# a-rtemis99/hpc_suffix_array

Measured on AMD Instinct MI355X. Metric: suffixes sorted/sec + ms/doubling-round, 1 GiB input at 1/2/4/8 MI355X, higher is better.
Workload: dtype u32

## Files before the change

### hpc_suffix_array_amd/_native.py

```python
from __future__ import annotations

import ctypes
import os
import subprocess

PKG_DIR = os.path.dirname(os.path.abspath(__file__))
LIB_PATH = os.path.join(PKG_DIR, "lib", "libsa_hip.so")
LIB_PATH = os.environ.get("SA_LIB_PATH", LIB_PATH)
CSRC = os.path.join(PKG_DIR, "csrc")

SA_MAX_ROUNDS = 64
KERNEL_KINDS = ["init", "hist_first", "hist_keys", "scan", "scatter_first", "scatter_keys",
                "heads", "heads_scan", "rerank", "seg_count", "seg_scan", "seg_write", "alphabet", "pack",
                "sort_u", "windows", "local_sort", "pivot_keys", "pivot_count", "pivot_write"]
SCHEDULE_PACKED = 0
SCHEDULE_REFERENCE = 1
ROUND1_AUTO = 0
ROUND1_LSD = 1
ROUND1_BUCKETED = 2
SA_K_COUNT = len(KERNEL_KINDS)
FIND_AUTO = 0
FIND_LANE = 1
FIND_WAVE = 2
FIND_LANE_MAX = 3584
# ... 5 lines not shown
LOCATE_TILE = 2048
LOCATE_ORDERS = {"text": 0, "sa": LOCATE_SA_ORDER}
MEM_INFO = 3
MEM_TOO_MANY = 1
MEM_LANE = 1
MEM_WAVE = 2
MEM_MODES = {"auto": 0, "lane": MEM_LANE, "wave": MEM_WAVE}

DROPIN_SYMBOLS = ["create_suffix_array", "destroy_suffix_array", "build_suffix_array",
                  "build_lcp_array", "find_longest_repeated_substring", "is_valid_suffix_array"]
EXT_SYMBOLS = ["sa_context_create", "sa_context_destroy", "sa_context_set_debug", "sa_workspace_bytes", "sa_build_device",
               "sa_build_ex", "sa_check_device", "sa_check", "sa_lcp_device", "sa_lcp", "sa_generate_text_device",
               "sa_alphabet_device", "sa_pack_keys_device", "sa_sort_pairs_device", "sa_scatter_u64_device",
               "sa_gather_u64_device", "sa_running_max_i64_device", "sa_inclusive_sum_i64_device",
               "sa_count_below_u64_device", "sa_select_u8_device",
               "sa_find_device", "sa_find", "sa_find_ex",
               "sa_match_device", "sa_matching_stats_device", "sa_match", "sa_matching_stats",
               "sa_bwt_device", "sa_bwt", "sa_inverse_device", "sa_inverse",
               "sa_locate_device", "sa_locate",
               "sa_mems_device", "sa_mems",
               "sa_dist_begin", "sa_dist_cuts", "sa_dist_plan_cuts", "sa_dist_reserve", "sa_dist_release", "sa_dist_round1", "sa_dist_req_count", "sa_dist_req_fill",
               "sa_dist_answer", "sa_dist_refine",
               "sa_last_error", "sa_host_syncs", "sa_device_count", "sa_version", "sa_struct_size"]


class SAError(RuntimeError):
    """A libsa_hip entry point returned an error code."""


DEBUG_FLAGS = {"no_cmp": 0x1, "no_pk8": 0x2, "no_pad": 0x4, "pad_overflow": 0x8, "no_fast32": 0x10,
               "no_pivot": 0x20, "perm_always": 0x40, "no_xq": 0x80, "xq_overflow": 0x100,
               "no_tied": 0x200, "no_key1_round": 0x400, "no_eonly": 0x800,
               "eonly": 0x1000, "fast32_small": 0x2000, "no_round2_fused": 0x4000,
               "ls_one_wg": 0x8000, "no_alpha_sample": 0x10000, "alpha_sample_small": 0x20000}


def debug_bits(names) -> int:
    bits = 0
    for x in names or ():
        if x not in DEBUG_FLAGS:
            raise ValueError(f"unknown debug flag {x!r} (one of {sorted(DEBUG_FLAGS)})")
        bits |= DEBUG_FLAGS[x]
    return bits


class SaOpts(ctypes.Structure):
    _fields_ = [("profile", ctypes.c_int32), ("schedule", ctypes.c_int32), ("init_chars", ctypes.c_int32),
                ("radix", ctypes.c_int32), ("round1", ctypes.c_int32), ("debug", ctypes.c_uint32),
                ("span_extra", ctypes.c_int32), ("tune", ctypes.c_int32)]


class SaStats(ctypes.Structure):
    _fields_ = [
        ("rounds", ctypes.c_int32),
        ("n_kinds", ctypes.c_int32),
        ("total_ms", ctypes.c_double),
        ("h2d_ms", ctypes.c_double),
        ("d2h_ms", ctypes.c_double),
        ("round_ms", ctypes.c_double * SA_MAX_ROUNDS),
        ("distinct", ctypes.c_uint64 * SA_MAX_ROUNDS),
        ("passes", ctypes.c_int32 * SA_MAX_ROUNDS),
        ("sorted_n", ctypes.c_uint64 * SA_MAX_ROUNDS),
        ("prefix_len", ctypes.c_uint64 * SA_MAX_ROUNDS),
        ("schedule", ctypes.c_int32),
        ("init_chars", ctypes.c_int32),
        ("sigma", ctypes.c_int32),
        ("sparse_ranks", ctypes.c_int32),
# ... 219 lines not shown
```

### hpc_suffix_array_amd/csrc/sa_build.hip

```cpp
#include <hip/hip_runtime.h>

#include <algorithm>
#include <atomic>
#include <chrono>
#include <cstdarg>
#include <cstdio>
#include <cstdlib>
#include <cstring>
#include <mutex>
#include <string>
#include <thread>
#include <vector>

#include "../../include/sa_hip.h"

#ifndef SA_ALPHA_GRID
#define SA_ALPHA_GRID 2048
#endif

#include "sa_bucket.h"
#include "sa_check.h"
#include "sa_kernels.h"
#include "sa_lcp.h"
#include "sa_limits.h"
// ... 1238 lines not shown
    const int r1 = opts ? opts->round1 : SA_ROUND1_AUTO;
    bool bucketed = false;
    auto plan_round1 = [&](bool sampled, bool* complete) -> int {
        SA_HIP(hipMemsetAsync(c->alpha, 0, 8 * 4, s));
        tm.begin(SA_K_ALPHABET);
        if (sampled) {
            const bool first4k = (c->dbg & SA_DEBUG_ALPHA_SAMPLE_SMALL) != 0;
            const uint64_t nb = alpha_text_blocks(n), ns = alpha_sample_blocks(n, first4k);
            hipLaunchKernelGGL(k_alphabet_sample, dim3((uint32_t)std::min<uint64_t>(ns, 2ull * (uint32_t)c->cus)),
                               dim3(kBlock), 0, s, d_text, n, nb, ns, c->alpha);
            add_bytes(st, SA_K_ALPHABET, alpha_sample_bytes(n, first4k));
        } else {
            const uint32_t grid = (uint32_t)std::min<uint64_t>((n + kBlock * 16 - 1) / (kBlock * 16), SA_ALPHA_GRID);
            hipLaunchKernelGGL(k_alphabet, dim3(grid), dim3(kBlock), 0, s, d_text, n, c->alpha);
            add_bytes(st, SA_K_ALPHABET, n);
        }
        tm.end();
        SA_HIP(hipGetLastError());
        SA_HIP(hipMemcpyAsync(h_alpha, c->alpha, 8 * 4, hipMemcpyDeviceToHost, s));
        SA_HIP(hipMemcpyAsync(h_tail, d_text + (n - tail_n), tail_n, hipMemcpyDeviceToHost, s));
        SA_HIP(host_sync(s));
        *complete = true;
        for (uint32_t t = 0; t < tail_n; ++t) {
            const uint32_t x = h_tail[t];
            if (!((h_alpha[x >> 5] >> (x & 31)) & 1u)) *complete = false;
            h_alpha[x >> 5] |= 1u << (x & 31);
        }
        sigma = 0;
        for (int b = 0; b < 256; ++b) h_code[b] = ((h_alpha[b >> 5] >> (b & 31)) & 1u) ? (uint16_t)(++sigma) : 0;
        SA_HIP(hipMemcpyAsync(c->code, h_code, 256 * 2, hipMemcpyHostToDevice, s));
        c->dna = sigma == 4 && h_code['A'] && h_code['C'] && h_code['G'] && h_code['T'];
        K = choose_chars(sigma, n, opts ? opts->init_chars : 0);
        Kb = (opts && opts->init_chars > 0) || sigma <= 1 ? K : min_chars(sigma, n);
        bucketed = plan_bucketed(sigma, n, Kb, r1, c->radix, &bp, 1, (c->dbg & SA_DEBUG_NO_CMP) ? 0 : 1);
        if (bucketed && bp.bs.cmp && short_suffix_ties(h_tail, n, tail_n, h_code, sigma, bp.bs.s, bp.bs.R))
            bucketed = plan_bucketed(sigma, n, Kb, r1, c->radix, &bp, 1, 0);
        const bool force_eonly = (c->dbg & SA_DEBUG_EONLY) != 0;
        if (bucketed && bp.bs.cmp == 1 && ((sigma & (sigma - 1)) != 0 || force_eonly) &&
            !(c->dbg & SA_DEBUG_NO_EONLY)) {
            const uint32_t hb = bp.bs.bb - kLoBits;
            BucketPlan b2;
            if ((force_eonly || !plan_pk8(bp, hb, c->dbg, true)) && plan_bucketed(sigma, n, Kb, r1, c->radix, &b2, 1, 2) &&
                (force_eonly || plan_pk8(b2, hb, c->dbg, true)) &&
                !short_suffix_ties(h_tail, n, tail_n, h_code, sigma, b2.bs.s, b2.bs.R, b2.K))
                bp = b2;
        }
        return SA_OK;
    };
    bool sampled = !(c->dbg & SA_DEBUG_NO_ALPHA_SAMPLE) &&
                   (n >= kPadMinN || (c->dbg & SA_DEBUG_ALPHA_SAMPLE_SMALL)) && c->radix == 0 && r1 != SA_ROUND1_LSD;
    bool refuted = false;
    uint64_t* keys1 = nullptr;
    uint32_t ksh1 = 0;
    uint32_t P = 0;
    bool fused = false;
    bool r1_pivot = false;
    uint64_t D = 0, m = 0, G = 0;
    uint64_t seg1[3] = {0, 0, 0};
    int r2 = 0;
    for (;;) {
        bool complete = true;
        rc = plan_round1(sampled, &complete);
        if (rc) return rc;
        if (sampled && !(bucketed && complete)) {
            SA_TRACE("packed: sampled alphabet (sigma=%u) not kept: %s", sigma,
                     complete ? "round 1 is not bucketed" : "the tail holds another symbol");
            sampled = false;
            continue;
        }
        c->samples_pending = false;
        if (!bucketed) break;
        bool done = false;
        c->alpha_prove = sampled && sigma < 256;
        c->alpha_refuted = false;
        rc = round1_bucketed(c, d_text, n, d_sa, bp, full_range(bp, n), s, tm, st, &done, &fused, seg1, &ksh1, true,
// ... 1057 lines not shown
```

### hpc_suffix_array_amd/csrc/sa_round1.h

```cpp
#pragma once

#ifndef SA_HIST_WPC
#define SA_HIST_WPC 64
#endif
#ifndef SA_REC_STRIPED
#define SA_REC_STRIPED 1
#endif
#ifndef SA_BB_EXTRA
#define SA_BB_EXTRA 0
#endif
#ifndef SA_ITEMS_A
#define SA_ITEMS_A 12
#endif
#ifndef SA_TEXT_BLOCK
#define SA_TEXT_BLOCK 512
#endif
#ifndef SA_LIST_BLOCK
#define SA_LIST_BLOCK 1024
#endif


#ifndef SA_SEG_BLOCK
#define SA_SEG_BLOCK 1024
#endif
// ... 26 lines not shown
    const uint32_t e = ((uint32_t)c->tune >> 8) & 0xFFu;
    const uint32_t v = e ? e : 8u;
    return v >= 8 ? 8u : v >= 4 ? 4u : v >= 2 ? 2u : 1u;
}

__global__ __launch_bounds__(kLoRadix) void k_sum_rows(const uint32_t* __restrict__ in, uint32_t rows,
                                                       uint32_t* __restrict__ out) {
    uint32_t t = 0;
    for (uint32_t r = 0; r < rows; ++r) t += in[r * kLoRadix + threadIdx.x];
    out[threadIdx.x] = t;
}
constexpr uint64_t kPadMaxN = 1ull << 31;
constexpr int kUsFlagWord = 12;
constexpr int kAlphaBadWord = 8;

static uint32_t key1_bits(const BucketSpec& bs) {
    unsigned __int128 dmax = 1;
    for (uint32_t t = 0; t < bs.s; ++t) dmax *= bs.sigma;
    const unsigned __int128 kmax = ((dmax - 1) << bs.rb) | (((unsigned __int128)1 << bs.rb) - 1);
    uint32_t kw = 0;
    for (unsigned __int128 x = kmax + 1; x; x >>= 1) ++kw;
    return kw;
}
constexpr uint32_t kPadStartOff = kLoRadix + 1024;
constexpr uint32_t kPadDenseOff = kPadStartOff + kLoRadix + 64;

struct BucketPlan {
    BucketSpec bs{};
    uint32_t ib = 0;
    uint32_t K = 0;
};

static bool plan_bucketed(uint32_t sigma, uint64_t n, uint32_t K, int round1, int radix, BucketPlan* p,
                          int world = 1, int cmp = 0) {
    if (round1 == SA_ROUND1_LSD || radix != 0 || sigma < 2 || n < 2) return false;
    if (round1 == SA_ROUND1_AUTO && n < kBucketMinN) return false;
    uint32_t bb = std::max<uint32_t>(16u, bit_width(n - 1) > 13 ? bit_width(n - 1) - 13 : 0u);
    if (world <= 1) bb = std::min<uint32_t>(bb, 18u);
    bb += SA_BB_EXTRA;
    if (bb > 18 + (uint32_t)bit_width((uint64_t)std::max(world, 1) - 1) || bb > 24) return false;
    uint64_t ps = 1;
    uint32_t s = 0;
    while (ps < (1ull << bb)) {
        ps *= sigma;
        ++s;
    }
    while (ps % (1ull << bb) != 0 && ps < (64ull << bb) && s + 1 < K && ps * sigma <= (1ull << 32)) {
        ps *= sigma;
        ++s;
    }
    if (ps > (1ull << 32)) return false;
    if (K <= s || K > (uint32_t)kMaxK) return false;
    const uint32_t ib = bit_width(n - 1);
    const uint32_t bd = bit_width(ps - 1);
    const uint32_t span = bit_width((ps + (1ull << bb) - 1) >> bb) + 1;
    for (uint32_t R = K - s; R >= 1; --R) {
        unsigned __int128 pr = 1;
        for (uint32_t t = 0; t < R; ++t) pr *= sigma;
        unsigned __int128 lowmax = cmp == 2 ? pr - 1 : cmp ? 2 * pr - 1 : s + (pr - 1) * (R + 1) + R;
        uint32_t rb = 0;
        while (lowmax) {
            ++rb;
            lowmax >>= 1;
        }
        if (bd + rb > 64 || rb + span + ib > 64) continue;
        p->bs.pow_s1 = ps / sigma;
        p->bs.powR1 = (uint64_t)(pr / sigma);
        p->bs.cmul = (1ull << 48) / ps;
        p->bs.bb = bb;
        p->bs.bsh = 48u - bb;
        p->bs.sigma = sigma;
        p->bs.s = s;
// ... 281 lines not shown
                               c->vals_alt, g_hi, cursor, m, blo, bhi, padded ? (const uint32_t*)pstart + 1 : nullptr,
                               padded ? c->words + 11 : nullptr, hb, bp.ib, stripes, alpha_bad);
        } else {
            SA_TEXT_PASS(false, false, kSpBlock, false, false);
        }
#undef SA_TEXT_PASS
    }
    tm.end();
    add_bytes(st, SA_K_SCATTER_FIRST, listed ? (pk8 ? 20 : 24) * m : n + (pk8 ? 8 : 12) * m);
    tm.begin(SA_K_SCAN);
    hipLaunchKernelGGL(k_digit_base_wide, dim3(1), dim3(1024), 0, s, (const uint32_t*)g_hi, 1u << hb,
                       os_base(c) + kLoRadix);
    if (xq)
        hipLaunchKernelGGL(k_xq_dh, dim3(1), dim3(1024), 0, s, (const uint32_t*)g_hi, 1u << hb,
                           (c->dbg & SA_DEBUG_XQ_OVERFLOW) ? 1u : 0u, xq_dh);
    if (padded) {
        if (stripes > 1)
            hipLaunchKernelGGL(k_sum_rows, dim3(1), dim3(kLoRadix), 0, s, (const uint32_t*)cursor, stripes, cursor_sum);
        hipLaunchKernelGGL(k_digit_base_wide, dim3(1), dim3(1024), 0, s, (const uint32_t*)cursor_sum, kLoRadix, dlo);
    }
    tm.end();
    tm.begin(SA_K_SCATTER_KEYS);
    {
        constexpr int kItemsB = SA_ITEMS_B, kItemsPk = SA_ITEMS_PK;
        const SrcBucketKeys sb{c->keys[0], c->vals_alt, bp.bs.rb, bp.bs.bsh, bp.bs.cmul, blo};
        const SrcPk8 sp{c->keys[0]};
        uint32_t* tk = os_tickets(c) + 1;
        const uint32_t* hbase = os_base(c) + kLoRadix;
        SA_HIP(hipMemsetAsync(c->segw, 0, segw_words(1u << hb) * 4, s));
        SegXq sx;
        if (xq) {
            SA_HIP(hipMemsetAsync(c->segx, 0, xqw * 4, s));
            sx.cur = c->segx;
            sx.sbase = reinterpret_cast<uint64_t*>(c->segx + (uint64_t)kXq * kSegs * (1u << hb));
            sx.done = c->segx + 3ull * kXq * kSegs * (1u << hb);
            sx.tickets = sx.done + kXq * kSegs;
            sx.dh = xq_dh;
            sx.err2 = c->words + 9;
            sx.cap = (uint32_t)std::min<uint64_t>(c->kucap, UINT32_MAX);
        }
        constexpr int kSegBlock = SA_SEG_BLOCK;
        const int sblk = hb <= 9 ? kSegBlock : kSpBlock;
        const uint64_t ut = (uint64_t)sblk * (pk8 ? kItemsPk : kItemsB);
        const uint64_t units = (m + ut - 1) / ut + kSegs;
        const uint32_t grid = xq ? (uint32_t)c->cus * (kSpBlock / sblk)
                                 : (uint32_t)std::max<uint64_t>(1, std::min<uint64_t>(units, (uint64_t)c->cus * (kSpBlock / sblk)));
        switch (hb) {
#define SA_SEG_LAUNCH(S, B, SRC, SH, IT)                                                                      \
    if (xq)                                                                                                   \
        hipLaunchKernelGGL((k_split_seg<S, B, IT, (B <= 9 ? kSegBlock : kSpBlock), true>), dim3(grid),        \
                           dim3(B <= 9 ? kSegBlock : kSpBlock), 0, s, SRC, m, SH,                              \
                           (const uint32_t*)(padded ? pstart : os_base(c)), hbase, c->segw, tk, bp.ib, c->keys_u,      \
                           c->words + 4, padded ? (const uint32_t*)cursor : nullptr,                           \
                           padded ? (const uint32_t*)dlo : nullptr, stripes, sx);                              \
    else                                                                                                      \
        hipLaunchKernelGGL((k_split_seg<S, B, IT, (B <= 9 ? kSegBlock : kSpBlock)>), dim3(grid),                \
                           dim3(B <= 9 ? kSegBlock : kSpBlock), 0, s, SRC, m, SH,                              \
                           (const uint32_t*)(padded ? pstart : os_base(c)), hbase, c->segw, tk, bp.ib, c->keys_u,      \
                           c->words + 4, padded ? (const uint32_t*)cursor : nullptr,                           \
                           padded ? (const uint32_t*)dlo : nullptr, stripes)
#define SA_SEG_PASS(B)                                                                                        \
    case B:                                                                                                   \
        if (pk8) SA_SEG_LAUNCH(SrcPk8, B, sp, 64u - B, kItemsPk);                                             \
        else SA_SEG_LAUNCH(SrcBucketKeys, B, sb, kLoBits, kItemsB);                                           \
        break;
            SA_SEG_PASS(7)
            SA_SEG_PASS(8)
            SA_SEG_PASS(9)
            SA_SEG_PASS(10)
#undef SA_SEG_PASS
#undef SA_SEG_LAUNCH
            default: return set_err(SA_E_INTERNAL, "second bucket pass of %u bits", hb);
        }
        const uint32_t gb = (uint32_t)std::min<uint64_t>(((uint64_t)nb_tab + kBlock) / kBlock, 1024);
        uint32_t* bstart = c->segw + kBstartOff;
        uint32_t* bdmin = bstart + kBstartWords;
#define SA_BSTARTS(R)                                                                                         \
    if (xq)                                                                                                   \
        hipLaunchKernelGGL(k_bucket_starts_xq<R>, dim3(R), dim3(kLoRadix), 0, s, hbase, (const uint32_t*)sx.cur, \
                           (const uint32_t*)xq_dh, m, bp.bs.cmul, bp.bs.bsh, bstart, bdmin, xq_pc, xq_pn, blo); \
    else                                                                                                      \
        hipLaunchKernelGGL(k_bucket_starts<R>, dim3(gb), dim3(kBlock), 0, s, (const uint32_t*)(padded ? dlo : os_base(c)), \
                           hbase, (const uint32_t*)c->segw, m, bp.bs.cmul, bp.bs.bsh, bstart, bdmin, blo)
        switch (hb) {
            case 7: SA_BSTARTS(128); break;
            case 8: SA_BSTARTS(256); break;
            case 9: SA_BSTARTS(512); break;
            default: SA_BSTARTS(1024); break;
        }
#undef SA_BSTARTS
    }
    tm.end();
    add_bytes(st, SA_K_SCATTER_KEYS, (pk8 ? 16 : 20) * m);
    SA_HIP(hipGetLastError());
    const uint64_t nw = (m + kWinStride - 1) / kWinStride;
    uint32_t* ws = c->vals_alt;
    uint32_t* list = c->vals_alt + nw + 1;
    tm.begin(SA_K_WINDOWS);
    {
        const uint32_t g1 = (uint32_t)std::min<uint64_t>((nw + kBlock) / kBlock, 8192);
        hipLaunchKernelGGL(k_window_starts_tab, dim3(g1), dim3(kBlock), 0, s, (const uint32_t*)(c->segw + kBstartOff),
                           nb_tab, m, nw, ws, list + 4 * nw + 2);
        const uint32_t g2 = (uint32_t)std::min<uint64_t>((nw + kBlock - 1) / kBlock, 1024);
        hipLaunchKernelGGL(k_window_list, dim3(g2), dim3(kBlock), 0, s, (const uint32_t*)ws, nw, list, c->words);
    }
    tm.end();
    add_bytes(st, SA_K_WINDOWS, 8 * nw);
    SA_HIP(hipGetLastError());
    SA_HIP(hipMemcpyAsync(c->host_words, c->words, 48, hipMemcpyDeviceToHost, s));
    uint32_t* skew = list + nw;
    uint32_t* cnt_u = skew + nw;
    uint32_t* cnt_g = cnt_u + nw + 1;
    uint32_t* const rank_arr = br_.rank ? br_.rank : c->rank;
// ... 208 lines not shown
```

### hpc_suffix_array_amd/csrc/sa_split.h

```cpp
#pragma once
#include <type_traits>
#include "sa_alpha.h"
#include "sa_bucket.h"
#include "sa_onesweep.h"

#ifndef SA_SEG_PROF
#define SA_SEG_PROF 0
#endif
#ifndef SA_TEXT_PROF
#define SA_TEXT_PROF 0
#endif

namespace sa {

constexpr int kSpBlock = 1024;
constexpr int kSpItems = 8;
constexpr int kSpTile = kSpBlock * kSpItems;
constexpr int kSpWaves = kSpBlock / kWave;

__device__ __forceinline__ uint32_t wave_min_u32(uint32_t x) {
#pragma unroll
    for (int o = kWave / 2; o > 0; o >>= 1) x = min(x, (uint32_t)__shfl_xor((int)x, o, kWave));
    return x;
}
__device__ __forceinline__ uint32_t wave_max_u32(uint32_t x) {
#pragma unroll
    for (int o = kWave / 2; o > 0; o >>= 1) x = max(x, (uint32_t)__shfl_xor((int)x, o, kWave));
    return x;
}

template <int RADIX, bool PROF = false, int kLook = 4>
__device__ __forceinline__ uint64_t tile_lookback(uint64_t* __restrict__ states, uint64_t t, uint32_t dg,
                                                  uint32_t tile_cnt, uint64_t tag, uint32_t* __restrict__ err,
                                                  uint32_t* steps = nullptr) {
    uint64_t excl = 0;
    if (t == 0) return 0;
    const uint32_t ep_now = (uint32_t)(tag >> 48) & kEpochMask;
// ... 815 lines not shown
                }
            }
        }
        __syncthreads();
#pragma unroll
        for (int j = 0; j < ITEMS; ++j) {
            const uint32_t q = j * BLOCK + dg;
            if (q < valid) {
                const uint64_t key = s_keys[q];
                const uint32_t dd =
                    PK8 ? s_pos[q] : (bucket_of(key, b.rb, b.cmul, b.bsh) - blo) & (RADIX - 1);
                const uint64_t g = (uint64_t)s_gofs[dd] + (q - s_start[dd]);
                if (g < m) {
                    out_keys[g] = key;
                    if constexpr (!PK8) out_vals[g] = s_pos[q];
                }
            }
        }
        __syncthreads();
#pragma unroll
        for (int j = 0; j < ITEMS; ++j) {
            k[j] = kn[j];
            v[j] = vn[j];
        }
        t = tn;
        tb = tbn;
        valid = validn;
        par ^= 1u;
    }
    for (uint32_t i = dg; i < 1024u; i += BLOCK)
        if (s_hhi[i]) atomicAdd(&ghist_hi[i], s_hhi[i]);
}

constexpr uint32_t kSegs = kLoRadix;
constexpr uint32_t kMaxStripes = 8;
constexpr uint64_t segw_words(int radix) { return 3ull * kSegs * radix + kSegs; }
constexpr uint64_t kBstartOff = segw_words(1024);
constexpr uint64_t kBstartWords = (1ull << 18) + 1;

constexpr uint32_t kXqSlack = 2048;
constexpr uint32_t kXqTicketStride = 32;
struct SegXq {
    uint32_t* cur = nullptr;
    uint64_t* sbase = nullptr;
    uint32_t* done = nullptr;
    uint32_t* tickets = nullptr;
    const uint32_t* dh = nullptr;
    uint32_t cap = 0;
    uint32_t* err2 = nullptr;
};
constexpr uint64_t xq_words(int radix) { return 3ull * kXq * kSegs * radix + kXq * kSegs + kXq * kXqTicketStride; }

template <class Src, int RBITS, int ITEMS, int BLOCK = kSpBlock, bool XQ = false>
__global__ __launch_bounds__(BLOCK, 2048 / BLOCK) void k_split_seg(Src src, uint64_t n, uint32_t shift,
                                                        const uint32_t* __restrict__ lo_base,
                                                        const uint32_t* __restrict__ digit_base,
                                                        uint32_t* __restrict__ segw, uint32_t* __restrict__ ticket,
                                                        uint32_t ib, uint64_t* __restrict__ out_w,
                                                        uint32_t* __restrict__ err,
                                                        const uint32_t* __restrict__ seg_cnt = nullptr,
                                                        const uint32_t* __restrict__ dense_lo = nullptr,
                                                        uint32_t stripes = 1, SegXq xq = SegXq{}) {
    constexpr int RADIX = 1 << RBITS;
    constexpr int RWAVES = RADIX / kWave;
    constexpr int WTILE = kWave * ITEMS;
    constexpr int TILE = BLOCK * ITEMS;
    static_assert(BLOCK >= RADIX && (int)kSegs <= BLOCK, "one thread per digit / segment");
    static_assert((int)(kSegs * kMaxStripes) <= 2 * BLOCK, "two sub-segments per thread in the unit numbering");
    static_assert(TILE <= 65535, "16-bit tile offsets");
    __shared__ uint64_t s_keys[TILE];
    __shared__ uint16_t s_dig[TILE];
    __shared__ uint32_t s_dmin[RADIX];
    __shared__ uint32_t s_cnt[RADIX];
    __shared__ uint16_t s_start[RADIX];
    __shared__ uint32_t s_gofs[RADIX];
    __shared__ uint32_t s_tmp[(BLOCK / kWave)];
    __shared__ uint32_t s_ubase[kSegs * kMaxStripes + 1];
    __shared__ uint32_t s_tile[2];
    __shared__ uint32_t s_last;
    __shared__ uint32_t s_claim[RADIX];
    const uint32_t xqq = XQ ? (blockIdx.x & (kXq - 1)) : 0u;
    uint32_t* const cur = XQ ? xq.cur + (uint64_t)xqq * kSegs * RADIX : segw;
    uint64_t* const sbase = XQ ? xq.sbase + (uint64_t)xqq * kSegs * RADIX
                               : reinterpret_cast<uint64_t*>(segw + (uint64_t)kSegs * RADIX);
    uint32_t* const done = XQ ? xq.done + xqq * kSegs : segw + 3ull * kSegs * RADIX;
    if constexpr (XQ) ticket = xq.tickets + xqq * kXqTicketStride;
    const uint64_t gcap = XQ ? (uint64_t)xq.cap : n;
    const uint32_t xrs = XQ ? xq.dh[RADIX] : 0u;
    constexpr uint64_t kReady = 1ull << 32;

    const uint32_t wave = wave_id(), lane = lane_id();
    const uint32_t dg = threadIdx.x;
    const uint32_t mask = RADIX - 1;
    const uint32_t nsub = kSegs * stripes;
    auto sub_lo = [&](uint32_t q) -> uint64_t {
        const uint32_t l = q / stripes, sidx = q % stripes;
        if (stripes == 1) return lo_base[l];
        return (uint64_t)lo_base[l] + sidx * ((lo_base[l + 1] - lo_base[l]) / stripes);
    };
    auto sub_hi = [&](uint32_t q) -> uint64_t {
        const uint32_t l = q / stripes, sidx = q % stripes;
        if (seg_cnt) return sub_lo(q) + seg_cnt[sidx * kSegs + l];
        return l + 1 < kSegs ? (uint64_t)lo_base[l + 1] : n;
    };
    const uint32_t* const dlo = dense_lo ? dense_lo : lo_base;
    {
        uint32_t x0 = 0, x1 = 0;
        const uint32_t q0 = 2 * dg, q1 = 2 * dg + 1;
        if (q0 < nsub) x0 = (uint32_t)((sub_hi(q0) - sub_lo(q0) + TILE - 1) / TILE);
        if (q1 < nsub) x1 = (uint32_t)((sub_hi(q1) - sub_lo(q1) + TILE - 1) / TILE);
        const uint32_t x = x0 + x1;
        const uint32_t inc = wave_inclusive_sum(x);
        if (lane == kWave - 1) s_tmp[wave] = inc;
        __syncthreads();
        uint32_t off = 0;
        for (uint32_t w = 0; w < wave; ++w) off += s_tmp[w];
        if (q0 < nsub) s_ubase[q0] = off + inc - x;
        if (q1 < nsub) s_ubase[q1] = off + inc - x1;
// ... 33 lines not shown
        }
    };
    uint32_t u = unit_of((uint32_t)__builtin_amdgcn_readfirstlane((int)s_tile[0]));
    uint32_t l = 0, valid = 0;
    uint64_t tb = 0;
    if (u < units) {
        locate(u, l, tb, valid);
        load(tb, valid, k, v);
    }
    uint32_t par = 0;
#if SA_SEG_PROF
    uint64_t pacc[7] = {0, 0, 0, 0, 0, 0, 0}, plast = clock64();
#define SEG_STAMP(k)                                \
    if (dg == 0) {                                  \
        const uint64_t now_ = clock64();            \
        pacc[k] += now_ - plast;                    \
        plast = now_;                               \
    }
#else
#define SEG_STAMP(k)
#endif
    while (u < units) {
        if (dg == 0) s_tile[par ^ 1u] = atomicAdd(ticket, 1u);
        uint32_t dr[ITEMS];
#pragma unroll
        for (int j = 0; j < ITEMS; ++j) {
            const uint32_t le = wave * WTILE + j * kWave + lane;
            const uint32_t d = le < valid ? src_digit(src, k[j], shift, mask, 0) : (uint32_t)RADIX;
            dr[j] = (d << 16) | (d < (uint32_t)RADIX ? atomicAdd(&s_cnt[d], 1u) : 0u);
        }
        __syncthreads();
        SEG_STAMP(0)
        uint32_t tile_cnt = 0;
        if (dg < (uint32_t)RADIX) {
            tile_cnt = s_cnt[dg];
            s_claim[dg] = tile_cnt ? atomicAdd(&cur[(uint64_t)l * RADIX + dg], tile_cnt) : 0u;
        }
        {
            const uint32_t x = (dg < (uint32_t)RADIX) ? tile_cnt : 0u;
            const uint32_t inc = wave_inclusive_sum(x);
            if (lane == kWave - 1 && wave < (uint32_t)RWAVES) s_tmp[wave] = inc;
            __syncthreads();
            uint32_t off = 0;
#pragma unroll
            for (int w = 0; w < RWAVES; ++w) off += (w < (int)wave) ? s_tmp[w] : 0u;
            if (dg < (uint32_t)RADIX) s_start[dg] = (uint16_t)(off + inc - x);
        }
        SEG_STAMP(1)
        if (dg == 0) s_last = atomicAdd(&done[l], 1u) == units_of(l) - 1 ? 1u : 0u;
        if (dg < (uint32_t)RADIX) {
            uint32_t bh;
            if (XQ ? qcount(s_ubase[l * stripes]) == 0 : dlo[l] == 0) {
                bh = XQ ? xqq * xrs + xq.dh[dg] : digit_base[dg];
            } else {
                uint64_t w;
                uint32_t spins = 0;
                while (((w = __hip_atomic_load(&sbase[(uint64_t)l * RADIX + dg], __ATOMIC_RELAXED,
                                               __HIP_MEMORY_SCOPE_AGENT)) & kReady) == 0) {
                    if (++spins > kSpinLimit) {
                        atomicOr(err, 1u);
                        break;
                    }
                    __builtin_amdgcn_s_sleep(1);
                }
                bh = (uint32_t)w;
            }
            s_gofs[dg] = bh + s_claim[dg];
            if constexpr (XQ) {
                if (tile_cnt && (uint64_t)bh + s_claim[dg] + tile_cnt > (uint64_t)xqq * xrs + xq.dh[dg + 1])
                    atomicOr(xq.err2, 1u);
            }
            s_claim[dg] = bh;
            if constexpr (!Src::kPk8) s_dmin[dg] = bucket_dmin(((dg << kLoBits) | l) + src.bofs, src.cmul, src.bsh);
        }
        __syncthreads();
        SEG_STAMP(2)
        if (s_last) {
            if (dg < (uint32_t)RADIX) {
                const uint32_t tot = __hip_atomic_load(&cur[(uint64_t)l * RADIX + dg], __ATOMIC_RELAXED,
                                                       __HIP_MEMORY_SCOPE_AGENT);
                for (uint32_t l2 = l + 1; l2 < kSegs; ++l2) {
                    __hip_atomic_store(&sbase[(uint64_t)l2 * RADIX + dg], kReady | (uint64_t)(s_claim[dg] + tot),
                                       __ATOMIC_RELAXED, __HIP_MEMORY_SCOPE_AGENT);
                    if (units_of(l2) > 0) break;
                }
            }
        }
        __syncthreads();
        const uint32_t un = unit_of((uint32_t)__builtin_amdgcn_readfirstlane((int)s_tile[par ^ 1u]));
        SEG_STAMP(3)
        uint32_t ln = l, validn = valid;
        uint64_t tbn = tb;
        if (un < units) locate(un, ln, tbn, validn);
        uint64_t kn[ITEMS];
        uint32_t vn[ITEMS];
        load(tbn, validn, kn, vn);
#pragma unroll
        for (int j = 0; j < ITEMS; ++j) {
            const uint32_t d = dr[j] >> 16;
            if (d < (uint32_t)RADIX) {
                const uint32_t pos = s_start[d] + (dr[j] & 0xFFFFu);
                if constexpr (Src::kPk8)
                    s_keys[pos] = k[j] & ((1ull << shift) - 1ull);
                else
                    s_keys[pos] = ((k[j] - ((uint64_t)s_dmin[d] << src.rb)) << ib) | v[j];
                s_dig[pos] = (uint16_t)d;
            }
        }
        __syncthreads();
        SEG_STAMP(4)
        if (dg < (uint32_t)RADIX) s_cnt[dg] = 0;
#pragma unroll
        for (int j = 0; j < ITEMS; ++j) {
            const uint32_t q = j * BLOCK + dg;
            if (q < valid) {
                const uint32_t dd = s_dig[q];
                const uint64_t g = (uint64_t)s_gofs[dd] + (q - s_start[dd]);
                if (g < gcap) out_w[g] = s_keys[q];
            }
        }
        __syncthreads();
        SEG_STAMP(5)
#pragma unroll
        for (int j = 0; j < ITEMS; ++j) {
            k[j] = kn[j];
            v[j] = vn[j];
        }
        u = un;
        l = ln;
        tb = tbn;
        valid = validn;
        par ^= 1u;
    }
#if SA_SEG_PROF
    if (dg == 0 && (blockIdx.x == 0 || blockIdx.x == gridDim.x / 2))
        printf("k_split_seg wg %u clk: rank %llu claim %llu base %llu ticket+load %llu scatter %llu write %llu\n",
               blockIdx.x, (unsigned long long)pacc[0], (unsigned long long)pacc[1], (unsigned long long)pacc[2],
               (unsigned long long)pacc[3], (unsigned long long)pacc[4], (unsigned long long)pacc[5]);
#endif
#undef SEG_STAMP
}

template <int RADIX>
__global__ __launch_bounds__(kBlock) void k_bucket_starts(const uint32_t* __restrict__ lo_base,
                                                          const uint32_t* __restrict__ digit_base,
                                                          const uint32_t* __restrict__ segw, uint64_t n,
                                                          uint64_t cmul, uint32_t bsh, uint32_t* __restrict__ bstart,
                                                          uint32_t* __restrict__ bdmin, uint32_t bofs) {
    const uint64_t* sbase = reinterpret_cast<const uint64_t*>(segw + (uint64_t)kSegs * RADIX);
    const uint32_t nb = (uint32_t)RADIX << kLoBits;
    for (uint32_t b = blockIdx.x * kBlock + threadIdx.x; b <= nb; b += gridDim.x * kBlock) {
        if (b == nb) {
            bstart[b] = (uint32_t)n;
            continue;
        }
        const uint32_t h = b >> kLoBits, l = b & (kSegs - 1);
        bstart[b] = lo_base[l] == 0 ? digit_base[h] : (uint32_t)sbase[(uint64_t)l * RADIX + h];
        bdmin[b] = bucket_dmin(b + bofs, cmul, bsh);
    }
}

__global__ __launch_bounds__(1024) void k_xq_dh(const uint32_t* __restrict__ tot, uint32_t radix, uint32_t exact_caps,
                                                uint32_t* __restrict__ dh) {
    __shared__ uint32_t s_tmp[1024 / kWave];
    const uint32_t t = threadIdx.x;
    uint32_t cap = 0;
    if (t < radix) {
        const uint32_t x = tot[t];
        cap = exact_caps ? x / kXq : x / kXq + x / 128u + kXqSlack;
    }
    const uint32_t inc = wave_inclusive_sum(cap);
    if (lane_id() == kWave - 1) s_tmp[wave_id()] = inc;
    __syncthreads();
    uint32_t off = 0;
    for (uint32_t w = 0; w < wave_id(); ++w) off += s_tmp[w];
    if (t < radix) dh[t] = off + inc - cap;
    if (t == radix - 1) dh[radix] = off + inc;
}

template <int RADIX>
__global__ __launch_bounds__(kLoRadix) void k_bucket_starts_xq(const uint32_t* __restrict__ digit_base,
                                                               const uint32_t* __restrict__ cur,
                                                               const uint32_t* __restrict__ dh,
                                                               uint64_t n, uint64_t cmul, uint32_t bsh,
                                                               uint32_t* __restrict__ bstart,
                                                               uint32_t* __restrict__ bdmin, uint32_t* __restrict__ pc,
                                                               uint32_t* __restrict__ pn, uint32_t bofs) {
    static_assert(kSegs == kLoRadix && kLoRadix % kWave == 0, "one thread per segment");
    __shared__ uint32_t s_tmp[kLoRadix / kWave];
    const uint32_t nb = (uint32_t)RADIX << kLoBits;
    const uint32_t h = blockIdx.x, l = threadIdx.x;
    const uint32_t b = (h << kLoBits) | l;
    auto excl = [&](uint32_t x) {
        const uint32_t inc = wave_inclusive_sum(x);
        __syncthreads();
        if (lane_id() == kWave - 1) s_tmp[wave_id()] = inc;
        __syncthreads();
        uint32_t off = 0;
        for (uint32_t w = 0; w < wave_id(); ++w) off += s_tmp[w];
        return off + inc - x;
    };
    const uint32_t rs = dh[RADIX];
    uint32_t tot = 0;
#pragma unroll 1
    for (uint32_t q = 0; q < kXq; ++q) {
        const uint32_t c = cur[((uint64_t)q * kSegs + l) * RADIX + h];
        tot += c;
        pn[(uint64_t)q * nb + b] = c;
        pc[(uint64_t)q * nb + b] = q * rs + dh[h] + excl(c);
    }
    bstart[b] = digit_base[h] + excl(tot);
    bdmin[b] = bucket_dmin(b + bofs, cmul, bsh);
    if (b == 0) bstart[nb] = (uint32_t)n;
}

}
```

### include/sa_hip.h

```cpp
#ifndef SA_HIP_H
#define SA_HIP_H

#include <stdint.h>

#ifdef __cplusplus
extern "C" {
#endif

#define SA_OK 0
#define SA_E_INVALID (-1)
#define SA_E_NOMEM (-2)
#define SA_E_HIP (-3)
#define SA_E_INTERNAL (-4)

#define SA_MAX_ROUNDS 64

enum sa_kernel_kind {
    SA_K_INIT = 0,
    SA_K_HIST_FIRST = 1,
    SA_K_HIST_KEYS = 2,
    SA_K_SCAN = 3,
    SA_K_SCATTER_FIRST = 4,
    SA_K_SCATTER_KEYS = 5,
    SA_K_HEADS = 6,
// ... 9 lines not shown
    SA_K_LOCAL_SORT = 16,
    SA_K_PIVOT_KEYS = 17,
    SA_K_PIVOT_COUNT = 18,
    SA_K_PIVOT_WRITE = 19,
    SA_K_COUNT = 20
};

#define SA_ROUND1_AUTO 0
#define SA_ROUND1_LSD 1
#define SA_ROUND1_BUCKETED 2
#define SA_ROUND1_PIVOT 3

#define SA_SCHEDULE_PACKED 0
#define SA_SCHEDULE_REFERENCE 1

#define SA_DEBUG_NO_CMP 0x1u
#define SA_DEBUG_NO_PK8 0x2u
#define SA_DEBUG_NO_PAD 0x4u
#define SA_DEBUG_PAD_OVERFLOW 0x8u
#define SA_DEBUG_NO_FAST32 0x10u
#define SA_DEBUG_NO_PIVOT 0x20u
#define SA_DEBUG_PERM_ALWAYS 0x40u
#define SA_DEBUG_NO_XQ 0x80u
#define SA_DEBUG_XQ_OVERFLOW 0x100u
#define SA_DEBUG_NO_KEY1_ROUND 0x400u
#define SA_DEBUG_NO_TIED 0x200u
#define SA_DEBUG_NO_EONLY 0x800u
#define SA_DEBUG_EONLY 0x1000u
#define SA_DEBUG_FAST32_SMALL 0x2000u
#define SA_DEBUG_NO_ROUND2_FUSED 0x4000u
#define SA_DEBUG_LS_ONE_WG 0x8000u
#define SA_DEBUG_NO_ALPHA_SAMPLE 0x10000u
#define SA_DEBUG_ALPHA_SAMPLE_SMALL 0x20000u

#define SA_ALPHABET_EXACT 0
#define SA_ALPHABET_SAMPLED 1
#define SA_ALPHABET_REFUTED 2

typedef struct {
    int32_t profile;
    int32_t schedule;
    int32_t init_chars;
    int32_t radix;
    int32_t round1;
    uint32_t debug;
    int32_t span_extra;
    int32_t tune;
} sa_opts;

typedef struct {
    int32_t rounds;
    int32_t n_kinds;
    double total_ms;
    double h2d_ms, d2h_ms;
    double round_ms[SA_MAX_ROUNDS];
    uint64_t distinct[SA_MAX_ROUNDS];
    int32_t passes[SA_MAX_ROUNDS];
    uint64_t sorted_n[SA_MAX_ROUNDS];
    uint64_t prefix_len[SA_MAX_ROUNDS];
    int32_t schedule;
    int32_t init_chars;
    int32_t sigma;
    int32_t sparse_ranks;
    int32_t round1;
    int32_t largest_window;
    uint64_t model_bytes;
// ... 167 lines not shown
```

Measured before the change: 112.2 billion.

## Pack segment claim count and tile count into one 64-bit atomic in split pass

The segmented split kernel now claims output space and counts finished tiles with a single 64-bit atomic per digit, which removes the separate done-counter atomic and one block barrier. The last claimant publishes the next segment base directly. The kernel also scans per-tile digit starts in a single wave with packed 16-bit stores, and precomputes per-digit write words so the scatter loop skips the digit array for pk8 keys. This costs extra cursor memory, adds an OLD template variant selectable via a tune bit, and adds a debug flag that enlarges the bucket bits.

```diff
diff --git a/hpc_suffix_array_amd/_native.py b/hpc_suffix_array_amd/_native.py
--- a/hpc_suffix_array_amd/_native.py
+++ b/hpc_suffix_array_amd/_native.py
@@ -61,7 +61,8 @@
                "no_pivot": 0x20, "perm_always": 0x40, "no_xq": 0x80, "xq_overflow": 0x100,
                "no_tied": 0x200, "no_key1_round": 0x400, "no_eonly": 0x800,
                "eonly": 0x1000, "fast32_small": 0x2000, "no_round2_fused": 0x4000,
-               "ls_one_wg": 0x8000, "no_alpha_sample": 0x10000, "alpha_sample_small": 0x20000}
+               "ls_one_wg": 0x8000, "no_alpha_sample": 0x10000, "alpha_sample_small": 0x20000,
+               "bb_plus1": 0x40000}
 
 
 def debug_bits(names) -> int:
diff --git a/hpc_suffix_array_amd/csrc/sa_build.hip b/hpc_suffix_array_amd/csrc/sa_build.hip
--- a/hpc_suffix_array_amd/csrc/sa_build.hip
+++ b/hpc_suffix_array_amd/csrc/sa_build.hip
@@ -1294,15 +1294,16 @@
         c->dna = sigma == 4 && h_code['A'] && h_code['C'] && h_code['G'] && h_code['T'];
         K = choose_chars(sigma, n, opts ? opts->init_chars : 0);
         Kb = (opts && opts->init_chars > 0) || sigma <= 1 ? K : min_chars(sigma, n);
-        bucketed = plan_bucketed(sigma, n, Kb, r1, c->radix, &bp, 1, (c->dbg & SA_DEBUG_NO_CMP) ? 0 : 1);
+        const uint32_t bbx = (c->dbg & SA_DEBUG_BB_PLUS1) ? 1u : 0u;
+        bucketed = plan_bucketed(sigma, n, Kb, r1, c->radix, &bp, 1, (c->dbg & SA_DEBUG_NO_CMP) ? 0 : 1, bbx);
         if (bucketed && bp.bs.cmp && short_suffix_ties(h_tail, n, tail_n, h_code, sigma, bp.bs.s, bp.bs.R))
-            bucketed = plan_bucketed(sigma, n, Kb, r1, c->radix, &bp, 1, 0);
+            bucketed = plan_bucketed(sigma, n, Kb, r1, c->radix, &bp, 1, 0, bbx);
         const bool force_eonly = (c->dbg & SA_DEBUG_EONLY) != 0;
         if (bucketed && bp.bs.cmp == 1 && ((sigma & (sigma - 1)) != 0 || force_eonly) &&
             !(c->dbg & SA_DEBUG_NO_EONLY)) {
             const uint32_t hb = bp.bs.bb - kLoBits;
             BucketPlan b2;
-            if ((force_eonly || !plan_pk8(bp, hb, c->dbg, true)) && plan_bucketed(sigma, n, Kb, r1, c->radix, &b2, 1, 2) &&
+            if ((force_eonly || !plan_pk8(bp, hb, c->dbg, true)) && plan_bucketed(sigma, n, Kb, r1, c->radix, &b2, 1, 2, bbx) &&
                 (force_eonly || plan_pk8(b2, hb, c->dbg, true)) &&
                 !short_suffix_ties(h_tail, n, tail_n, h_code, sigma, b2.bs.s, b2.bs.R, b2.K))
                 bp = b2;
diff --git a/hpc_suffix_array_amd/csrc/sa_round1.h b/hpc_suffix_array_amd/csrc/sa_round1.h
--- a/hpc_suffix_array_amd/csrc/sa_round1.h
+++ b/hpc_suffix_array_amd/csrc/sa_round1.h
@@ -82,12 +82,12 @@
 };
 
 static bool plan_bucketed(uint32_t sigma, uint64_t n, uint32_t K, int round1, int radix, BucketPlan* p,
-                          int world = 1, int cmp = 0) {
+                          int world = 1, int cmp = 0, uint32_t bb_extra = 0) {
     if (round1 == SA_ROUND1_LSD || radix != 0 || sigma < 2 || n < 2) return false;
     if (round1 == SA_ROUND1_AUTO && n < kBucketMinN) return false;
     uint32_t bb = std::max<uint32_t>(16u, bit_width(n - 1) > 13 ? bit_width(n - 1) - 13 : 0u);
     if (world <= 1) bb = std::min<uint32_t>(bb, 18u);
-    bb += SA_BB_EXTRA;
+    bb += SA_BB_EXTRA + bb_extra;
     if (bb > 18 + (uint32_t)bit_width((uint64_t)std::max(world, 1) - 1) || bb > 24) return false;
     uint64_t ps = 1;
     uint32_t s = 0;
@@ -435,8 +435,8 @@
         if (xq) {
             SA_HIP(hipMemsetAsync(c->segx, 0, xqw * 4, s));
             sx.cur = c->segx;
-            sx.sbase = reinterpret_cast<uint64_t*>(c->segx + (uint64_t)kXq * kSegs * (1u << hb));
-            sx.done = c->segx + 3ull * kXq * kSegs * (1u << hb);
+            sx.sbase = reinterpret_cast<uint64_t*>(c->segx + (uint64_t)kSegCurWords * kXq * kSegs * (1u << hb));
+            sx.done = c->segx + (kSegCurWords + 2ull) * kXq * kSegs * (1u << hb);
             sx.tickets = sx.done + kXq * kSegs;
             sx.dh = xq_dh;
             sx.err2 = c->words + 9;
@@ -448,24 +448,23 @@
         const uint64_t units = (m + ut - 1) / ut + kSegs;
         const uint32_t grid = xq ? (uint32_t)c->cus * (kSpBlock / sblk)
                                  : (uint32_t)std::max<uint64_t>(1, std::min<uint64_t>(units, (uint64_t)c->cus * (kSpBlock / sblk)));
+        const bool seg_old = (((uint32_t)c->tune >> 31) & 1u) != 0;
         switch (hb) {
+#define SA_SEG_LAUNCH2(S, B, SRC, SH, IT, XQF, OLDF)                                                          \
+    hipLaunchKernelGGL((k_split_seg<S, B, IT, (B <= 9 ? kSegBlock : kSpBlock), XQF, OLDF>), dim3(grid),       \
+                       dim3(B <= 9 ? kSegBlock : kSpBlock), 0, s, SRC, m, SH,                                  \
+                       (const uint32_t*)(padded ? pstart : os_base(c)), hbase, c->segw, tk, bp.ib, c->keys_u,  \
+                       c->words + 4, padded ? (const uint32_t*)cursor : nullptr,                               \
+                       padded ? (const uint32_t*)dlo : nullptr, stripes, sx)
 #define SA_SEG_LAUNCH(S, B, SRC, SH, IT)                                                                      \
-    if (xq)                                                                                                   \
-        hipLaunchKernelGGL((k_split_seg<S, B, IT, (B <= 9 ? kSegBlock : kSpBlock), true>), dim3(grid),        \
-                           dim3(B <= 9 ? kSegBlock : kSpBlock), 0, s, SRC, m, SH,                              \
-                           (const uint32_t*)(padded ? pstart : os_base(c)), hbase, c->segw, tk, bp.ib, c->keys_u,      \
-                           c->words + 4, padded ? (const uint32_t*)cursor : nullptr,                           \
-                           padded ? (const uint32_t*)dlo : nullptr, stripes, sx);                              \
-    else                                                                                                      \
-        hipLaunchKernelGGL((k_split_seg<S, B, IT, (B <= 9 ? kSegBlock : kSpBlock)>), dim3(grid),                \
-                           dim3(B <= 9 ? kSegBlock : kSpBlock), 0, s, SRC, m, SH,                              \
-                           (const uint32_t*)(padded ? pstart : os_base(c)), hbase, c->segw, tk, bp.ib, c->keys_u,      \
-                           c->words + 4, padded ? (const uint32_t*)cursor : nullptr,                           \
-                           padded ? (const uint32_t*)dlo : nullptr, stripes)
+    if (xq && seg_old) SA_SEG_LAUNCH2(S, B, SRC, SH, IT, true, true);                                         \
+    else if (xq) SA_SEG_LAUNCH2(S, B, SRC, SH, IT, true, false);                                              \
+    else if (seg_old) SA_SEG_LAUNCH2(S, B, SRC, SH, IT, false, true);                                         \
+    else SA_SEG_LAUNCH2(S, B, SRC, SH, IT, false, false)
 #define SA_SEG_PASS(B)                                                                                        \
     case B:                                                                                                   \
-        if (pk8) SA_SEG_LAUNCH(SrcPk8, B, sp, 64u - B, kItemsPk);                                             \
-        else SA_SEG_LAUNCH(SrcBucketKeys, B, sb, kLoBits, kItemsB);                                           \
+        if (pk8) { SA_SEG_LAUNCH(SrcPk8, B, sp, 64u - B, kItemsPk); }                                         \
+        else { SA_SEG_LAUNCH(SrcBucketKeys, B, sb, kLoBits, kItemsB); }                                       \
         break;
             SA_SEG_PASS(7)
             SA_SEG_PASS(8)
@@ -473,6 +472,7 @@
             SA_SEG_PASS(10)
 #undef SA_SEG_PASS
 #undef SA_SEG_LAUNCH
+#undef SA_SEG_LAUNCH2
             default: return set_err(SA_E_INTERNAL, "second bucket pass of %u bits", hb);
         }
         const uint32_t gb = (uint32_t)std::min<uint64_t>(((uint64_t)nb_tab + kBlock) / kBlock, 1024);
@@ -481,7 +481,7 @@
 #define SA_BSTARTS(R)                                                                                         \
     if (xq)                                                                                                   \
         hipLaunchKernelGGL(k_bucket_starts_xq<R>, dim3(R), dim3(kLoRadix), 0, s, hbase, (const uint32_t*)sx.cur, \
-                           (const uint32_t*)xq_dh, m, bp.bs.cmul, bp.bs.bsh, bstart, bdmin, xq_pc, xq_pn, blo); \
+                           (seg_old ? 1u : kSegCurWords), (const uint32_t*)xq_dh, m, bp.bs.cmul, bp.bs.bsh, bstart, bdmin, xq_pc, xq_pn, blo); \
     else                                                                                                      \
         hipLaunchKernelGGL(k_bucket_starts<R>, dim3(gb), dim3(kBlock), 0, s, (const uint32_t*)(padded ? dlo : os_base(c)), \
                            hbase, (const uint32_t*)c->segw, m, bp.bs.cmul, bp.bs.bsh, bstart, bdmin, blo)
diff --git a/hpc_suffix_array_amd/csrc/sa_seg_cursor.h b/hpc_suffix_array_amd/csrc/sa_seg_cursor.h
--- /dev/null
+++ b/hpc_suffix_array_amd/csrc/sa_seg_cursor.h
@@ -0,0 +1,27 @@
+#pragma once
+#include <stdint.h>
+
+#if defined(__HIPCC__) || defined(__HIP__)
+#define SA_SEG_HD __host__ __device__ __forceinline__
+#else
+#define SA_SEG_HD inline
+#endif
+
+namespace sa {
+
+SA_SEG_HD uint64_t seg_claim_add(uint32_t cnt) { return (1ull << 32) | cnt; }
+SA_SEG_HD uint32_t seg_claim_items(uint64_t old) { return (uint32_t)old; }
+SA_SEG_HD uint32_t seg_claim_count(uint64_t old) { return (uint32_t)(old >> 32); }
+SA_SEG_HD bool seg_claim_last(uint64_t old, uint32_t units) { return seg_claim_count(old) == units - 1u; }
+SA_SEG_HD uint32_t seg_claim_total(uint64_t old, uint32_t cnt) { return seg_claim_items(old) + cnt; }
+
+constexpr uint32_t kSegTabSkip = ~0u;
+SA_SEG_HD uint32_t seg_tab_word(uint32_t base, uint32_t claim, uint32_t start, uint32_t cnt, uint64_t end, bool* fits) {
+    const uint64_t g0 = (uint64_t)base + claim;
+    const uint32_t w = (uint32_t)g0 - start;
+    *fits = g0 + cnt <= end && w != kSegTabSkip;
+    return *fits ? w : kSegTabSkip;
+}
+SA_SEG_HD uint32_t seg_tab_place(uint32_t word, uint32_t q) { return word + q; }
+
+}
diff --git a/hpc_suffix_array_amd/csrc/sa_split.h b/hpc_suffix_array_amd/csrc/sa_split.h
--- a/hpc_suffix_array_amd/csrc/sa_split.h
+++ b/hpc_suffix_array_amd/csrc/sa_split.h
@@ -3,6 +3,7 @@
 #include "sa_alpha.h"
 #include "sa_bucket.h"
 #include "sa_onesweep.h"
+#include "sa_seg_cursor.h"
 
 #ifndef SA_SEG_PROF
 #define SA_SEG_PROF 0
@@ -884,9 +885,20 @@
         if (s_hhi[i]) atomicAdd(&ghist_hi[i], s_hhi[i]);
 }
 
+#ifndef SA_SEG_CNT64
+#define SA_SEG_CNT64 1
+#endif
+#ifndef SA_SEG_TAB1
+#define SA_SEG_TAB1 1
+#endif
+#ifndef SA_SEG_SCAN1
+#define SA_SEG_SCAN1 1
+#endif
 constexpr uint32_t kSegs = kLoRadix;
 constexpr uint32_t kMaxStripes = 8;
-constexpr uint64_t segw_words(int radix) { return 3ull * kSegs * radix + kSegs; }
+constexpr uint32_t kSegCurWords = SA_SEG_CNT64 ? 2 : 1;
+constexpr uint64_t seg_base_off(int radix) { return (uint64_t)kSegCurWords * kSegs * radix; }
+constexpr uint64_t segw_words(int radix) { return (kSegCurWords + 2ull) * kSegs * radix + kSegs; }
 constexpr uint64_t kBstartOff = segw_words(1024);
 constexpr uint64_t kBstartWords = (1ull << 18) + 1;
 
@@ -901,9 +913,11 @@
     uint32_t cap = 0;
     uint32_t* err2 = nullptr;
 };
-constexpr uint64_t xq_words(int radix) { return 3ull * kXq * kSegs * radix + kXq * kSegs + kXq * kXqTicketStride; }
-
-template <class Src, int RBITS, int ITEMS, int BLOCK = kSpBlock, bool XQ = false>
+constexpr uint64_t xq_words(int radix) {
+    return (kSegCurWords + 2ull) * kXq * kSegs * radix + kXq * kSegs + kXq * kXqTicketStride;
+}
+
+template <class Src, int RBITS, int ITEMS, int BLOCK = kSpBlock, bool XQ = false, bool OLD = false>
 __global__ __launch_bounds__(BLOCK, 2048 / BLOCK) void k_split_seg(Src src, uint64_t n, uint32_t shift,
                                                         const uint32_t* __restrict__ lo_base,
                                                         const uint32_t* __restrict__ digit_base,
@@ -920,11 +934,16 @@
     static_assert(BLOCK >= RADIX && (int)kSegs <= BLOCK, "one thread per digit / segment");
     static_assert((int)(kSegs * kMaxStripes) <= 2 * BLOCK, "two sub-segments per thread in the unit numbering");
     static_assert(TILE <= 65535, "16-bit tile offsets");
+    constexpr bool CNT64 = !OLD && SA_SEG_CNT64 != 0;
+    constexpr bool TAB1 = !OLD && SA_SEG_TAB1 != 0, SCAN1 = !OLD && SA_SEG_SCAN1 != 0;
+    constexpr bool PKW = TAB1 && Src::kPk8;
+    constexpr int CPL = RADIX / kWave;
+    static_assert(CPL >= 2 && CPL % 2 == 0, "SCAN1 packs two 16-bit starts per word");
     __shared__ uint64_t s_keys[TILE];
-    __shared__ uint16_t s_dig[TILE];
+    __shared__ uint16_t s_dig[PKW ? 2 : TILE];
     __shared__ uint32_t s_dmin[RADIX];
-    __shared__ uint32_t s_cnt[RADIX];
-    __shared__ uint16_t s_start[RADIX];
+    __shared__ __attribute__((aligned(16))) uint32_t s_cnt[RADIX];
+    __shared__ __attribute__((aligned(16))) uint16_t s_start[RADIX];
     __shared__ uint32_t s_gofs[RADIX];
     __shared__ uint32_t s_tmp[(BLOCK / kWave)];
     __shared__ uint32_t s_ubase[kSegs * kMaxStripes + 1];
@@ -932,10 +951,11 @@
     __shared__ uint32_t s_last;
     __shared__ uint32_t s_claim[RADIX];
     const uint32_t xqq = XQ ? (blockIdx.x & (kXq - 1)) : 0u;
-    uint32_t* const cur = XQ ? xq.cur + (uint64_t)xqq * kSegs * RADIX : segw;
+    uint32_t* const cur = XQ ? xq.cur + (uint64_t)xqq * kSegs * RADIX * kSegCurWords : segw;
+    unsigned long long* const cur64 = reinterpret_cast<unsigned long long*>(cur);
     uint64_t* const sbase = XQ ? xq.sbase + (uint64_t)xqq * kSegs * RADIX
-                               : reinterpret_cast<uint64_t*>(segw + (uint64_t)kSegs * RADIX);
-    uint32_t* const done = XQ ? xq.done + xqq * kSegs : segw + 3ull * kSegs * RADIX;
+                               : reinterpret_cast<uint64_t*>(segw + seg_base_off(RADIX));
+    uint32_t* const done = XQ ? xq.done + xqq * kSegs : segw + (kSegCurWords + 2ull) * kSegs * RADIX;
     if constexpr (XQ) ticket = xq.tickets + xqq * kXqTicketStride;
     const uint64_t gcap = XQ ? (uint64_t)xq.cap : n;
     const uint32_t xrs = XQ ? xq.dh[RADIX] : 0u;
@@ -1035,11 +1055,39 @@
         __syncthreads();
         SEG_STAMP(0)
         uint32_t tile_cnt = 0;
+        unsigned long long clw = 0;
         if (dg < (uint32_t)RADIX) {
             tile_cnt = s_cnt[dg];
-            s_claim[dg] = tile_cnt ? atomicAdd(&cur[(uint64_t)l * RADIX + dg], tile_cnt) : 0u;
-        }
-        {
+            if constexpr (CNT64)
+                clw = atomicAdd(&cur64[(uint64_t)l * RADIX + dg], (unsigned long long)seg_claim_add(tile_cnt));
+            else
+                s_claim[dg] = tile_cnt ? atomicAdd(&cur[(uint64_t)l * RADIX + dg], tile_cnt) : 0u;
+        }
+        if constexpr (SCAN1) {
+            if (wave == 0) {
+                uint32_t c[CPL];
+                if constexpr (CPL % 4 == 0) {
+#pragma unroll
+                    for (int i = 0; i < CPL / 4; ++i) {
+                        const uint4 c4 = *reinterpret_cast<const uint4*>(&s_cnt[CPL * lane + 4 * i]);
+                        c[4 * i] = c4.x, c[4 * i + 1] = c4.y, c[4 * i + 2] = c4.z, c[4 * i + 3] = c4.w;
+                    }
+                } else {
+                    const uint2 c2 = *reinterpret_cast<const uint2*>(&s_cnt[CPL * lane]);
+                    c[0] = c2.x, c[1] = c2.y;
+                }
+                uint32_t sum = 0;
+#pragma unroll
+                for (int i = 0; i < CPL; ++i) sum += c[i];
+                uint32_t e = wave_inclusive_sum(sum) - sum;
+                uint32_t* const st32 = reinterpret_cast<uint32_t*>(&s_start[CPL * lane]);
+#pragma unroll
+                for (int i = 0; i < CPL; i += 2) {
+                    st32[i / 2] = e | ((e + c[i]) << 16);
+                    e += c[i] + c[i + 1];
+                }
+            }
+        } else {
             const uint32_t x = (dg < (uint32_t)RADIX) ? tile_cnt : 0u;
             const uint32_t inc = wave_inclusive_sum(x);
             if (lane == kWave - 1 && wave < (uint32_t)RWAVES) s_tmp[wave] = inc;
@@ -1050,7 +1098,10 @@
             if (dg < (uint32_t)RADIX) s_start[dg] = (uint16_t)(off + inc - x);
         }
         SEG_STAMP(1)
-        if (dg == 0) s_last = atomicAdd(&done[l], 1u) == units_of(l) - 1 ? 1u : 0u;
+        if constexpr (!CNT64) {
+            if (dg == 0) s_last = atomicAdd(&done[l], 1u) == units_of(l) - 1 ? 1u : 0u;
+        }
+        uint32_t run_base = 0, run_claim = 0;
         if (dg < (uint32_t)RADIX) {
             uint32_t bh;
             if (XQ ? qcount(s_ubase[l * stripes]) == 0 : dlo[l] == 0) {
@@ -1068,28 +1119,64 @@
                 }
                 bh = (uint32_t)w;
             }
-            s_gofs[dg] = bh + s_claim[dg];
-            if constexpr (XQ) {
-                if (tile_cnt && (uint64_t)bh + s_claim[dg] + tile_cnt > (uint64_t)xqq * xrs + xq.dh[dg + 1])
-                    atomicOr(xq.err2, 1u);
-            }
-            s_claim[dg] = bh;
+            const uint32_t claim = CNT64 ? seg_claim_items(clw) : s_claim[dg];
+            if constexpr (TAB1) {
+                run_base = bh;
+                run_claim = claim;
+            } else {
+                s_gofs[dg] = bh + claim;
+                if constexpr (XQ) {
+                    if (tile_cnt && (uint64_t)bh + claim + tile_cnt > (uint64_t)xqq * xrs + xq.dh[dg + 1])
+                        atomicOr(xq.err2, 1u);
+                }
+            }
+            if constexpr (CNT64) {
+                if (seg_claim_last(clw, units_of(l))) {
+                    const uint32_t nb = bh + seg_claim_total(clw, tile_cnt);
+                    for (uint32_t l2 = l + 1; l2 < kSegs; ++l2) {
+                        __hip_atomic_store(&sbase[(uint64_t)l2 * RADIX + dg], kReady | (uint64_t)nb, __ATOMIC_RELAXED,
+                                           __HIP_MEMORY_SCOPE_AGENT);
+                        if (units_of(l2) > 0) break;
+                    }
+                }
+            } else {
+                s_claim[dg] = bh;
+            }
             if constexpr (!Src::kPk8) s_dmin[dg] = bucket_dmin(((dg << kLoBits) | l) + src.bofs, src.cmul, src.bsh);
         }
         __syncthreads();
         SEG_STAMP(2)
-        if (s_last) {
+        if constexpr (SCAN1) {
+            if (dg < (uint32_t)RADIX) s_cnt[dg] = 0;
+        }
+        if constexpr (TAB1) {
             if (dg < (uint32_t)RADIX) {
-                const uint32_t tot = __hip_atomic_load(&cur[(uint64_t)l * RADIX + dg], __ATOMIC_RELAXED,
-                                                       __HIP_MEMORY_SCOPE_AGENT);
-                for (uint32_t l2 = l + 1; l2 < kSegs; ++l2) {
-                    __hip_atomic_store(&sbase[(uint64_t)l2 * RADIX + dg], kReady | (uint64_t)(s_claim[dg] + tot),
-                                       __ATOMIC_RELAXED, __HIP_MEMORY_SCOPE_AGENT);
-                    if (units_of(l2) > 0) break;
-                }
-            }
-        }
-        __syncthreads();
+                uint64_t end = gcap;
+                if constexpr (XQ) {
+                    const uint64_t send = (uint64_t)xqq * xrs + xq.dh[dg + 1];
+                    end = send < end ? send : end;
+                }
+                bool fits;
+                s_gofs[dg] = seg_tab_word(run_base, run_claim, s_start[dg], tile_cnt, end, &fits);
+                if constexpr (XQ) {
+                    if (tile_cnt && !fits) atomicOr(xq.err2, 1u);
+                }
+            }
+        }
+        if constexpr (!CNT64) {
+            if (s_last) {
+                if (dg < (uint32_t)RADIX) {
+                    const uint32_t tot = __hip_atomic_load(&cur[(uint64_t)l * RADIX + dg], __ATOMIC_RELAXED,
+                                                           __HIP_MEMORY_SCOPE_AGENT);
+                    for (uint32_t l2 = l + 1; l2 < kSegs; ++l2) {
+                        __hip_atomic_store(&sbase[(uint64_t)l2 * RADIX + dg], kReady | (uint64_t)(s_claim[dg] + tot),
+                                           __ATOMIC_RELAXED, __HIP_MEMORY_SCOPE_AGENT);
+                        if (units_of(l2) > 0) break;
+                    }
+                }
+            }
+            __syncthreads();
+        }
         const uint32_t un = unit_of((uint32_t)__builtin_amdgcn_readfirstlane((int)s_tile[par ^ 1u]));
         SEG_STAMP(3)
         uint32_t ln = l, validn = valid;
@@ -1103,23 +1190,35 @@
             const uint32_t d = dr[j] >> 16;
             if (d < (uint32_t)RADIX) {
                 const uint32_t pos = s_start[d] + (dr[j] & 0xFFFFu);
-                if constexpr (Src::kPk8)
+                if constexpr (PKW)
+                    s_keys[pos] = k[j];
+                else if constexpr (Src::kPk8)
                     s_keys[pos] = k[j] & ((1ull << shift) - 1ull);
                 else
                     s_keys[pos] = ((k[j] - ((uint64_t)s_dmin[d] << src.rb)) << ib) | v[j];
-                s_dig[pos] = (uint16_t)d;
+                if constexpr (!PKW) s_dig[pos] = (uint16_t)d;
             }
         }
         __syncthreads();
         SEG_STAMP(4)
-        if (dg < (uint32_t)RADIX) s_cnt[dg] = 0;
+        if constexpr (!SCAN1) {
+            if (dg < (uint32_t)RADIX) s_cnt[dg] = 0;
+        }
+        const uint64_t lowmask = (1ull << shift) - 1ull;
 #pragma unroll
         for (int j = 0; j < ITEMS; ++j) {
             const uint32_t q = j * BLOCK + dg;
             if (q < valid) {
-                const uint32_t dd = s_dig[q];
-                const uint64_t g = (uint64_t)s_gofs[dd] + (q - s_start[dd]);
-                if (g < gcap) out_w[g] = s_keys[q];
+                if constexpr (TAB1) {
+                    const uint64_t key = s_keys[q];
+                    const uint32_t dd = PKW ? (uint32_t)(key >> shift) : (uint32_t)s_dig[q];
+                    const uint32_t gw = s_gofs[dd];
+                    if (gw != kSegTabSkip) out_w[seg_tab_place(gw, q)] = PKW ? key & lowmask : key;
+                } else {
+                    const uint32_t dd = s_dig[q];
+                    const uint64_t g = (uint64_t)s_gofs[dd] + (q - s_start[dd]);
+                    if (g < gcap) out_w[g] = s_keys[q];
+                }
             }
         }
         __syncthreads();
@@ -1150,7 +1249,7 @@
                                                           const uint32_t* __restrict__ segw, uint64_t n,
                                                           uint64_t cmul, uint32_t bsh, uint32_t* __restrict__ bstart,
                                                           uint32_t* __restrict__ bdmin, uint32_t bofs) {
-    const uint64_t* sbase = reinterpret_cast<const uint64_t*>(segw + (uint64_t)kSegs * RADIX);
+    const uint64_t* sbase = reinterpret_cast<const uint64_t*>(segw + seg_base_off(RADIX));
     const uint32_t nb = (uint32_t)RADIX << kLoBits;
     for (uint32_t b = blockIdx.x * kBlock + threadIdx.x; b <= nb; b += gridDim.x * kBlock) {
         if (b == nb) {
@@ -1183,7 +1282,7 @@
 
 template <int RADIX>
 __global__ __launch_bounds__(kLoRadix) void k_bucket_starts_xq(const uint32_t* __restrict__ digit_base,
-                                                               const uint32_t* __restrict__ cur,
+                                                               const uint32_t* __restrict__ cur, uint32_t cw,
                                                                const uint32_t* __restrict__ dh,
                                                                uint64_t n, uint64_t cmul, uint32_t bsh,
                                                                uint32_t* __restrict__ bstart,
@@ -1207,7 +1306,7 @@
     uint32_t tot = 0;
 #pragma unroll 1
     for (uint32_t q = 0; q < kXq; ++q) {
-        const uint32_t c = cur[((uint64_t)q * kSegs + l) * RADIX + h];
+        const uint32_t c = cur[(((uint64_t)q * kSegs * kSegCurWords + (uint64_t)l * cw) * RADIX + (uint64_t)h * cw)];
         tot += c;
         pn[(uint64_t)q * nb + b] = c;
         pc[(uint64_t)q * nb + b] = q * rs + dh[h] + excl(c);
diff --git a/include/sa_hip.h b/include/sa_hip.h
--- a/include/sa_hip.h
+++ b/include/sa_hip.h
@@ -65,6 +65,7 @@
 #define SA_DEBUG_LS_ONE_WG 0x8000u
 #define SA_DEBUG_NO_ALPHA_SAMPLE 0x10000u
 #define SA_DEBUG_ALPHA_SAMPLE_SMALL 0x20000u
+#define SA_DEBUG_BB_PLUS1 0x40000u
 
 #define SA_ALPHABET_EXACT 0
 #define SA_ALPHABET_SAMPLED 1
```

Measured after the change: 112.7 billion (median of 6 runs). Within noise of the previous version (+0.4%).
